# mtumalan/VisionTransformer

Measured on AMD Instinct MI355X. Metric: images/sec (512×512) ViT-B/16 seg, 1/2/4/8 MI355X + mask argmax match, higher is better.
Workload: dtype f32

## Files before the change

### visiontransformer_amd/csrc/common.hpp

```cpp
#pragma once
#include <hip/hip_runtime.h>
#include <stdint.h>

#include "../../include/vitseg.h"

namespace vitseg {

constexpr int WAVE = 64;

typedef float f32x4 __attribute__((ext_vector_type(4)));
typedef float f32x16 __attribute__((ext_vector_type(16)));
typedef short bf16x8 __attribute__((ext_vector_type(8)));
typedef short bf16x4 __attribute__((ext_vector_type(4)));

void set_error(const char* fmt, ...);
int hip_fail(hipError_t e, const char* what);

enum Opt {
    OPT_NO_F32P = 0,
    OPT_NO_P8,
    OPT_NO_H16P,
    OPT_NO_RAGGED_P8,
    OPT_NO_DROPMASK,
    OPT_DROPW_LIMIT_MB,
    OPT_UPSAMPLE_GLOBAL,
    OPT_BF16_TILES,
    OPT_F32P_NOINL,
    OPT_GN,
    OPT_NO_MASK2,
    OPT_NO_SMALL,
    OPT_SMALL_VARIANT,
    OPT_SMALL_MAX_ROWS,
    OPT_CONV_DMA,
    OPT_COUNT
};
long opt(int id);

#define VITSEG_CHECK_ARG(cond, code, ...) \
    do {                                  \
        if (!(cond)) {                    \
            ::vitseg::set_error(__VA_ARGS__); \
            return (code);                \
        }                                 \
    } while (0)

#define VITSEG_LAUNCH_CHECK(what)                               \
    do {                                                        \
        hipError_t e__ = hipGetLastError();                     \
        if (e__ != hipSuccess) return ::vitseg::hip_fail(e__, what); \
    } while (0)

inline size_t up256(size_t v) { return (v + 255) & ~(size_t)255; }

__device__ __forceinline__ int xcd_remap(int bid, int nwg) {
    const int q = nwg >> 3, r = nwg & 7, xcd = bid & 7, idx = bid >> 3;
    const int base = (xcd < r) ? xcd * (q + 1) : r * (q + 1) + (xcd - r) * q;
    return base + idx;
}

struct AttnTile {
    int rt, head, b;
};
__device__ __forceinline__ AttnTile attn_tile(int ntiles, int A) {
    const int t = xcd_remap(blockIdx.x, gridDim.x);
    const int bh = t / ntiles;
    AttnTile r;
// ... 118 lines not shown
#endif
__device__ __forceinline__ int wave_sum(int v) {
    for (int d = WAVE / 2; d > 0; d >>= 1) v += __shfl_xor(v, d);
    return v;
}

__device__ __forceinline__ float gelu_phi(float u) {
#pragma clang fp contract(off)
    const float a = fabsf(u) * 0.70710678118654752440f;
    const float c = fminf(a, 5.0f);
    float q = __uint_as_float(0xb6e5811du);
    q = fmaf(c, q, __uint_as_float(0x38d55d79u));
    q = fmaf(c, q, __uint_as_float(0xba2329bbu));
    q = fmaf(c, q, __uint_as_float(0x3ae4efa2u));
    q = fmaf(c, q, __uint_as_float(0x3a233c25u));
    q = fmaf(c, q, __uint_as_float(0xbce796e6u));
    q = fmaf(c, q, __uint_as_float(0x3e181a64u));
    q = fmaf(c, q, __uint_as_float(0x3f6b1c07u));
    q = fmaf(c, q, __uint_as_float(0x3fd05f5fu));
    const float e = __builtin_amdgcn_exp2f(-(a * q));
    return u >= 0.f ? fmaf(e, -0.5f, 1.0f) : 0.5f * e;
}
__device__ __forceinline__ float gelu_erf(float u) {
#pragma clang fp contract(off)
    return u * gelu_phi(u);
}

__device__ __forceinline__ float gelu_erf_grad(float u) {
#pragma clang fp contract(off)
    const float pdf = __builtin_amdgcn_exp2f((u * u) * -0.72134752044448170368f);
    return fmaf(u * pdf, 0.39894228040143267794f, gelu_phi(u));
}

__device__ __forceinline__ float gelu_erf_fast(float u) {
    const float x = fabsf(u) * 0.70710678118654752440f;
    float t = fmaf(x, 0.0000430638f, 0.0002765672f);
    t = fmaf(x, t, 0.0001520143f);
    t = fmaf(x, t, 0.0092705272f);
    t = fmaf(x, t, 0.0422820123f);
    t = fmaf(x, t, 0.0705230784f);
    t = fmaf(x, t, 1.0f);
    t = t * t;
    t = t * t;
    t = t * t;
    t = t * t;
    const float erf_abs = 1.0f - __builtin_amdgcn_rcpf(t);
    return 0.5f * u + 0.5f * fabsf(u) * erf_abs;
}
struct GeluPair {
    float g, d;
};
__device__ __forceinline__ GeluPair gelu_erf_pair_fast(float u) {
    const float a = fabsf(u) * 0.70710678118654752440f;
    const float c = fminf(a, 4.5f);
    float q = __uint_as_float(0xb98ef51du);
    q = fmaf(c, q, __uint_as_float(0x3b8f4085u));
    q = fmaf(c, q, __uint_as_float(0xbd04359fu));
    q = fmaf(c, q, __uint_as_float(0x3e1a8172u));
    q = fmaf(c, q, __uint_as_float(0x3f6af0d8u));
    q = fmaf(c, q, __uint_as_float(0x3fd0616eu));
    const float e = __builtin_amdgcn_exp2f(-(a * q));
    const float phi = u >= 0.f ? fmaf(e, -0.5f, 1.0f) : 0.5f * e;
    const float pdf = __builtin_amdgcn_exp2f((u * u) * -0.72134752044448170368f);
    return GeluPair{u * phi, fmaf(u * pdf, 0.39894228040143267794f, phi)};
}

__device__ __forceinline__ unsigned short f32_to_bf16(float f) {
    unsigned u = __float_as_uint(f);
    if ((u & 0x7fffffffu) > 0x7f800000u) return (unsigned short)((u >> 16) | 0x40);
    return (unsigned short)((u + 0x7fffu + ((u >> 16) & 1u)) >> 16);
}
__device__ __forceinline__ unsigned pack2_bf16(float lo, float hi) {
    typedef __bf16 bf16v2_t __attribute__((ext_vector_type(2)));
    typedef float f32v2_t __attribute__((ext_vector_type(2)));
    const f32v2_t f = {lo, hi};
    return __builtin_bit_cast(unsigned, __builtin_convertvector(f, bf16v2_t));
}
__device__ __forceinline__ float bf16_to_f32(unsigned short h) { return __uint_as_float(((unsigned)h) << 16); }

typedef unsigned short bf16_t;
// ... 31 lines not shown
```

### visiontransformer_amd/csrc/gemm_dispatch.hip

```cpp
#include "gemm_tiles.hpp"

namespace vitseg {
namespace {

int whole_split_shape(int M, int N, int K, int kstep) { return K % kstep == 0 ? whole_split(M, N, K, kstep) : 0; }

int thin_slices(int K, int kstep) {
    if (K < 256 || K % kstep != 0) return 0;
    const int sl = K / kstep / 4;
    return sl > THIN_MAX_SPLITS ? THIN_MAX_SPLITS : sl < 1 ? 1 : sl;
}

int whole_split_applies(const GemmArgs& a, int epi, int kstep) {
    const int sp = whole_split_shape(a.M, a.N, a.K, kstep);
    const bool ok = sp && a.thin_scratch && (size_t)sp * a.M * a.N <= a.thin_capacity && !a.drop.thresh &&
                    !a.aux && a.splitk <= 1 && a.ldc % 4 == 0 && (epi == EPI_BIAS || epi == EPI_GELU || epi == EPI_RESADD);
    return ok ? sp : 0;
}

int thin_split_applies(const GemmArgs& a, int epi, int kstep) {
    const bool h16 = kstep == 64;
    const int sl = thin_slices(a.K, kstep);
    const bool ok = sl && a.thin_scratch && a.thin_rows > 0 && a.thin_rows <= THIN_MAX_ROWS && a.M > a.thin_rows &&
                    (size_t)sl * a.thin_rows * a.N <= a.thin_capacity && (a.M - a.thin_rows) % BM == 0 &&
                    (h16 || (!a.drop.thresh && !a.aux)) && a.splitk <= 1 && a.ldc % 4 == 0 &&
                    (epi == EPI_BIAS || epi == EPI_GELU || epi == EPI_RESADD || (h16 && epi == EPI_DGELU));
    return ok ? sl : 0;
}

template <typename F>
int sliced(GemmArgs a, int splits, float* scratch, hipStream_t s, F launch) {
    float* out = (float*)a.C;
    if (splits > 1) {
        a.C = scratch;
        a.splitk = splits;
    }
    a.split_stride = (size_t)a.M * a.N;
    if (int rc = launch(a)) return rc;
    return splits > 1 ? launch_splitk_reduce(scratch, out, (size_t)a.M * a.N / 4, splits, s) : VITSEG_OK;
}

enum H16Kernel { HK_NONE, HK_TILE, HK_LARGE, HK_XL, HK_P8, HK_H16P };

struct H16Route {
    H16Kernel body;
    int body_rows;
    int tail_rows;
    int slices;
    int colsum_rows;
};

}

int launch_gemm_f32(const GemmArgs& a_in, int amode, int epi, hipStream_t s, int x3) {
    if (x3 != 1 && x3 != 2) x3 = 0;
    GemmArgs a = a_in;
    if (amode == A_PLAIN) {
        if (const int sp = whole_split_applies(a_in, epi, 32)) {
            a.thin_rows = a_in.M;
            return launch_thin_rows(GT_F32, x3, a, epi, sp, s);
        }
        if (const int sl = thin_split_applies(a_in, epi, 32)) {
            if (int rc = launch_thin_rows(GT_F32, x3, a_in, epi, sl, s)) return rc;
            a.M = a_in.M - a_in.thin_rows;
        }
    }
    a.thin_scratch = nullptr;
    VITSEG_CHECK_ARG(a.M > 0 && a.N > 0 && a.K > 0 && a.K % 4 == 0, VITSEG_EINVAL, "gemm_f32: bad M/N/K %d %d %d", a.M, a.N, a.K);
    VITSEG_CHECK_ARG(a.N % 4 == 0 && a.ldc % 4 == 0, VITSEG_ESHAPE, "gemm: N=%d and ldc=%d must be multiples of 4", a.N, a.ldc);
    if (amode == A_PLAIN) {
        VITSEG_CHECK_ARG(a.lda % 4 == 0, VITSEG_EINVAL, "gemm_f32: lda %% 4");
        if (!x3 && gemm_f32p_applies(a, epi)) return launch_gemm_f32p(a, epi, s);
    } else if (amode == A_PATCH && epi == EPI_POS) {
        VITSEG_CHECK_ARG(a.P % 4 == 0, VITSEG_ESHAPE, "patch size must be a multiple of 4");
    } else if (amode == A_CONV3 && epi == EPI_RELU) {
        VITSEG_CHECK_ARG(a.D % 4 == 0, VITSEG_ESHAPE, "hidden size must be a multiple of 4");
    }
    static const char* const who[3] = {"gemm_f32", "gemm_f32 (x3)", "gemm_f32 (x3, split W)"};
    return launch_gemm_tile(GT_F32, true, amode, epi, x3, a, s, who[x3]);
}

int launch_gemm_f32_bwd(const GemmArgs& a, int amode, int ta, int tb, int epi, hipStream_t s) {
    VITSEG_CHECK_ARG(a.M > 0 && a.N > 0 && a.K > 0, VITSEG_EINVAL, "gemm_bwd: bad M/N/K %d %d %d", a.M, a.N, a.K);
    VITSEG_CHECK_ARG(a.N % 4 == 0 && a.ldc % 4 == 0 && a.lda % 4 == 0 && a.ldw % 4 == 0, VITSEG_ESHAPE,
                     "gemm_bwd: leading dimensions must be multiples of 4");
    VITSEG_CHECK_ARG(ta || a.K % 4 == 0, VITSEG_ESHAPE, "gemm_bwd: K %% 4");
    VITSEG_CHECK_ARG(!ta || a.M % 4 == 0, VITSEG_ESHAPE, "gemm_bwd: M %% 4 for a T-form A");
    return launch_gemm_tile_bwd(amode, ta, tb, epi, a, s);
}

int launch_wgrad_f32(GemmArgs a, float* scratch, hipStream_t s) {
    const int splits = wgrad_splits(a.M, a.N, a.K, 32);
    VITSEG_CHECK_ARG(splits <= 1 || (a.ldc == a.N && scratch), VITSEG_EINVAL, "wgrad: split-K needs a dense output and scratch");
    return sliced(a, splits, scratch, s, [&](const GemmArgs& g) { return launch_gemm_f32_bwd(g, A_PLAIN, 1, 1, EPI_BIAS, s); });
}

static int route_h16(const GemmArgs& a_in, int amode, int epi, H16Route& r) {
    r = H16Route{HK_NONE, 0, 0, 0, 0};
    const bool want_cs = a_in.colsum_out && a_in.colsum_scratch && epi == EPI_DGELU;
    const auto persistent = [&](const GemmArgs& g) {
        r.body = gemm_h16p_applies(g, epi) ? HK_H16P : HK_P8;
        r.body_rows = g.M;
        r.colsum_rows = want_cs ? g.M : 0;
        return VITSEG_OK;
    };
    GemmArgs a = a_in;
    if (amode == A_PLAIN) {
        if (const int sp = whole_split_applies(a_in, epi, 64)) {
            r.tail_rows = a_in.M;
            r.slices = sp;
            return VITSEG_OK;
        }
        if (a_in.M % 256 != 0 && a_in.M % 256 <= 128 && gemm_p8_applies(a_in, epi) &&
            gemm_p8_rounds(a_in.M, a_in.N) == gemm_p8_rounds(a_in.M - a_in.M % 256, a_in.N) && !opt(OPT_NO_RAGGED_P8))
            return persistent(a_in);
        const int sl = (a_in.M - a_in.thin_rows) % LBM == 0 ? thin_split_applies(a_in, epi, 64) : 0;
        if (sl) {
            r.tail_rows = a_in.thin_rows;
            r.slices = sl;
            a.M = a_in.M - a_in.thin_rows;
        }
    }
    VITSEG_CHECK_ARG(a.M > 0 && a.N > 0 && a.K > 0, VITSEG_EINVAL, "gemm_bf16: bad M/N/K %d %d %d", a.M, a.N, a.K);
    VITSEG_CHECK_ARG(a.K % 64 == 0, VITSEG_ESHAPE, "gemm_bf16: K=%d must be a multiple of 64", a.K);
    VITSEG_CHECK_ARG(a.N % 4 == 0 && a.ldc % 4 == 0, VITSEG_ESHAPE, "gemm: N=%d and ldc=%d must be multiples of 4", a.N, a.ldc);
    if (amode == A_PLAIN && gemm_p8_applies(a, epi)) {
        const int tail = a.M % 256;
        if (tail != 0 && tail <= 128) {
            r.tail_rows = tail;
            a.M -= tail;
        }
        return persistent(a);
    }
    const long force = opt(OPT_BF16_TILES);
    const bool xl = force ? force == 3 : (a.M >= 8192 && a.N >= 2048);
    const bool large = force ? force == 2 : (!xl && a.M >= 4096 && a.K >= 2048);
    r.body_rows = a.M;
    if (amode == A_PLAIN) {
        VITSEG_CHECK_ARG(a.lda % 8 == 0, VITSEG_EINVAL, "gemm_bf16: lda %% 8");
        r.body = xl ? HK_XL : large ? HK_LARGE : HK_TILE;
        if (epi == EPI_BIAS || epi == EPI_GELU || epi == EPI_DGELU || epi == EPI_RESADD) return VITSEG_OK;
    } else if (amode == A_CONV3 && (epi == EPI_RELU || epi == EPI_BIAS)) {
        VITSEG_CHECK_ARG(a.D % 64 == 0 && a.zeros, VITSEG_ESHAPE, "%s must be a multiple of 64",
                         epi == EPI_RELU ? "hidden size" : "channel count");
        r.body = large ? HK_LARGE : HK_TILE;
        return VITSEG_OK;
    }
    set_error("gemm_bf16: unsupported amode/epilogue %d/%d", amode, epi);
    return VITSEG_EINVAL;
}

int launch_gemm_bf16(const GemmArgs& a_in, int amode, int epi, hipStream_t s, bool f16) {
    H16Route r;
    if (int rc = route_h16(a_in, amode, epi, r)) return rc;
    const GemmType type = f16 ? GT_F16 : GT_BF16;
    const bool out_f32 = epi == EPI_RESADD || amode == A_CONV3;
    GemmArgs a = a_in;
    if (r.slices) {
        a.thin_rows = r.tail_rows;
        if (int rc = launch_thin_rows(type, 0, a, epi, r.slices, s)) return rc;
    }
    a.M = r.body_rows;
    a.thin_scratch = nullptr;
    if (!r.colsum_rows) a.colsum_scratch = nullptr;
    int rc = VITSEG_OK;
    switch (r.body) {
        case HK_NONE: break;
        case HK_P8: rc = launch_gemm_p8(a, epi, s, f16); break;
        case HK_H16P: rc = launch_gemm_h16p(a, s, f16); break;
        case HK_XL: rc = launch_gemm_large(f16, amode, epi, 256, a, s, "gemm_bf16"); break;
        case HK_LARGE: rc = launch_gemm_large(f16, amode, epi, 128, a, s, "gemm_bf16"); break;
        case HK_TILE: rc = launch_gemm_tile(type, out_f32, amode, epi, 0, a, s, "gemm_bf16");
    }
    if (rc) return rc;
    if (r.tail_rows && !r.slices) {
        GemmArgs t = a;
        const auto row = [&](const void* p, size_t esz) { return (char*)p + (size_t)r.body_rows * a.ldc * esz; };
        t.M = r.tail_rows;
        t.row_base = a.row_base + r.body_rows;
        t.A = (const char*)a.A + (size_t)r.body_rows * a.lda * 2;
        if (a.aux) t.aux = row(a.aux, 2);
        if (a.R) t.R = (const float*)row(a.R, epi == EPI_RESADD ? 4 : 2);
        t.C = row(a.C, out_f32 ? 4 : 2);
        if ((rc = launch_gemm_tile(type, out_f32, A_PLAIN, epi, 0, t, s, "gemm_bf16"))) return rc;
    }
    if (!a_in.colsum_out) return VITSEG_OK;
    VITSEG_CHECK_ARG(a_in.colsum_scratch && !f16, VITSEG_EINVAL, "gemm: column sums need bf16 + scratch");
    if (r.colsum_rows > 0)
        return launch_colsum_finish_fused((const bf16_t*)a_in.C + (size_t)r.colsum_rows * a_in.ldc, a_in.M - r.colsum_rows,
                                          2 * ((r.colsum_rows + 255) / 256), a_in.colsum_out, a_in.colsum_scratch, a_in.N,
                                          a_in.ldc, s);
    return launch_colsum(a_in.C, 1, a_in.colsum_out, a_in.colsum_scratch, a_in.M, a_in.N, a_in.ldc, s);
}
// ... 37 lines not shown
```

### visiontransformer_amd/csrc/gemm_tile.hip

```cpp
#include "gemm_tiles.hpp"

namespace vitseg {
namespace {

template <typename T> struct Elem;
template <> struct Elem<float> { static constexpr int CE = 4, BKE = 32; };
template <> struct Elem<bf16_t> { static constexpr int CE = 8, BKE = 64; };
template <> struct Elem<f16_t> { static constexpr int CE = 8, BKE = 64; };

template <typename T>
struct ARow {
    const T* base;
    int y, x;
    bool valid;
};

template <typename T, int AMODE>
__device__ __forceinline__ ARow<T> make_arow(const GemmArgs& p, int m) {
    ARow<T> r;
    r.valid = m < p.M;
    r.y = r.x = 0;
    const T* A = (const T*)p.A;
    if (!r.valid) {
        r.base = A;
// ... 134 lines not shown
                wrow[i] = (const T*)p.W + (size_t)(wvalid[i] ? n : 0) * p.ldw;
            }
        }
        const bool ta_col_ok = m0 + tc * 4 < p.M, tb_col_ok = n0 + tc * 4 < p.N;
        f32x4 ra[4], rb[4];
        bool oka[4], okb[4];
        auto gload = [&](int kt) {
            const int k = (kt + kt0) * BKE + lc * CE;
            const int kc = min(k, p.K - CE);
#pragma unroll
            for (int i = 0; i < 4; ++i) {
                if constexpr (TA) {
                    const int kr = (kt + kt0) * BKE + tr + 8 * i;
                    oka[i] = ta_col_ok && kr < p.K;
                    ra[i] = *(const f32x4*)((const T*)p.A + (size_t)(oka[i] ? kr : 0) * p.lda +
                                            (oka[i] ? m0 + tc * 4 : 0));
                } else {
                    ra[i] = load_a<T, AMODE>(p, arow[i], k, oka[i]);
                }
                if constexpr (TB) {
                    const int kr = (kt + kt0) * BKE + tr + 8 * i;
                    okb[i] = tb_col_ok && kr < p.K;
                    rb[i] = *(const f32x4*)((const T*)p.W + (size_t)(okb[i] ? kr : 0) * p.ldw +
                                            (okb[i] ? n0 + tc * 4 : 0));
                } else {
                    rb[i] = *(const f32x4*)(wrow[i] + kc);
                    okb[i] = wvalid[i] && k < p.K;
                }
            }
        };
        const int wpos = lr * BK + ((lc ^ ((lr >> 1) & 7)) << 2);
        const int tpos = tr * BM + tc * 4;
        const int xpos = lr * 16 + ((((lc >> 1) ^ ((lr >> 1) & 3)) << 2) | ((lc & 1) << 1));
        auto split = [&](const f32x4& v, uint2& hi, uint2& lo) {
            const _Float16 h0 = (_Float16)v[0], h1 = (_Float16)v[1], h2 = (_Float16)v[2], h3 = (_Float16)v[3];
            hi.x = __builtin_bit_cast(unsigned, f16x2{h0, h1});
            hi.y = __builtin_bit_cast(unsigned, f16x2{h2, h3});
            lo.x = H16<f16_t>::pack2((v[0] - (float)h0) * 2048.f, (v[1] - (float)h1) * 2048.f);
            lo.y = H16<f16_t>::pack2((v[2] - (float)h2) * 2048.f, (v[3] - (float)h3) * 2048.f);
        };
        auto swrite = [&](int buf) {
            const f32x4 z = {0.f, 0.f, 0.f, 0.f};
#pragma unroll
            for (int i = 0; i < 4; ++i) {
                if constexpr (X3) {
                    uint2 hi, lo;
                    split(oka[i] ? ra[i] : z, hi, lo);
                    *(uint2*)&lds[buf][0][xpos + 32 * i * 16] = hi;
                    *(uint2*)&lds[buf][0][2048 + xpos + 32 * i * 16] = lo;
                    if constexpr (X3 == 2) {
                        const f32x4 w = okb[i] ? rb[i] : z;
                        hi = uint2{__float_as_uint(w[0]), __float_as_uint(w[1])};
                        lo = uint2{__float_as_uint(w[2]), __float_as_uint(w[3])};
                    } else {
                        split(okb[i] ? rb[i] : z, hi, lo);
                    }
                    *(uint2*)&lds[buf][1][xpos + 32 * i * 16] = hi;
                    *(uint2*)&lds[buf][1][2048 + xpos + 32 * i * 16] = lo;
                } else {
                    *(f32x4*)&lds[buf][0][TA ? tpos + 8 * i * BM : wpos + 32 * i * BK] = oka[i] ? ra[i] : z;
                    *(f32x4*)&lds[buf][1][TB ? tpos + 8 * i * BN : wpos + 32 * i * BK] = okb[i] ? rb[i] : z;
                }
            }
        };
        if constexpr (X3) {
            f32x4 ah[2][MI], al[2][MI], bh[2][NI], bl[2][NI];
            const int xsw = (li >> 1) & 3;
            auto lfragx = [&](int buf, int st, int slot) {
                const int ch = ((2 * st + lh) ^ xsw) << 2;
#pragma unroll
                for (int mi = 0; mi < MI; ++mi) {
                    const float* r = &lds[buf][0][(a_row0 + li + mi * 32) * 16 + ch];
                    ah[slot][mi] = *(const f32x4*)r;
                    al[slot][mi] = *(const f32x4*)(r + 2048);
                }
#pragma unroll
                for (int ni = 0; ni < NI; ++ni) {
                    const float* r = &lds[buf][1][(b_col0 + li + ni * 32) * 16 + ch];
                    bh[slot][ni] = *(const f32x4*)r;
                    bl[slot][ni] = *(const f32x4*)(r + 2048);
                }
            };
            auto mfmax = [&](int slot) {
#pragma unroll
                for (int mi = 0; mi < MI; ++mi)
#pragma unroll
                    for (int ni = 0; ni < NI; ++ni) {
                        const bf16x8 xh = __builtin_bit_cast(bf16x8, ah[slot][mi]), xl = __builtin_bit_cast(bf16x8, al[slot][mi]);
// ... 243 lines not shown
    else if (rows_valid <= 64)
        gemm_tile<T, OutT, AMODE, EPI, 2, 1, TA, TB, X3>(p, lds, m0, n0, 0, wave * 32);
    else
        gemm_tile<T, OutT, AMODE, EPI, 2, 2, TA, TB, X3>(p, lds, m0, n0, (wave >> 1) * 64, (wave & 1) * 64);
}

template <typename T, typename OutT, int AMODE, int EPI, int TA = 0, int TB = 0, int X3 = 0>
int launch_one(GemmArgs a, hipStream_t s) {
    if (a.ldw == 0) a.ldw = TB ? a.N : a.K;
    if (!a.gn) a.gn = env_gn();
    const int tiles = ((a.M + BM - 1) / BM) * ((a.N + BN - 1) / BN);
    const int splits = a.splitk > 1 ? a.splitk : 1;
    hipLaunchKernelGGL((gemm_kernel<T, OutT, AMODE, EPI, TA, TB, X3>), dim3(tiles, splits), dim3(256), 0, s, a);
    VITSEG_LAUNCH_CHECK("gemm");
    return VITSEG_OK;
}

template <int EPI, typename OutT>
__global__ __launch_bounds__(256) void thin_reduce_kernel(const float* __restrict__ partial, const float* __restrict__ bias,
                                                          const float* __restrict__ R, OutT* __restrict__ C, int rows, int N,
                                                          int ldc, int splits, OutT* __restrict__ aux, DropArgs drop,
                                                          unsigned row0) {
    const int n4 = N >> 2;
    const int i = blockIdx.x * 256 + threadIdx.x;
    if (i >= rows * n4) return;
    const int r = i / n4, c = (i - r * n4) * 4;
    const size_t slab = (size_t)rows * N;
    f32x4 acc = *(const f32x4*)(partial + (size_t)r * N + c);
    for (int sIdx = 1; sIdx < splits; ++sIdx) {
        const f32x4 v = *(const f32x4*)(partial + sIdx * slab + (size_t)r * N + c);
#pragma unroll
        for (int e = 0; e < 4; ++e) acc[e] += v[e];
    }
    f32x4 b4 = {0.f, 0.f, 0.f, 0.f};
    if (bias) b4 = *(const f32x4*)(bias + c);
    f32x4 res = {0.f, 0.f, 0.f, 0.f};
    if (EPI == EPI_RESADD) res = *(const f32x4*)(R + (size_t)r * ldc + c);
    if constexpr (EPI == EPI_DGELU) {
        const uint2 d = *(const uint2*)((const OutT*)R + (size_t)r * ldc + c);
        res[0] = H16<OutT>::lo(d.x);
        res[1] = H16<OutT>::hi(d.x);
        res[2] = H16<OutT>::lo(d.y);
        res[3] = H16<OutT>::hi(d.y);
    }
    f32x4 der = {0.f, 0.f, 0.f, 0.f};
    const unsigned key = drop.thresh ? drop_key(drop.seed, drop.stream, row0 + (unsigned)r) : 0u;
#pragma unroll
    for (int e = 0; e < 4; ++e) {
        float x = acc[e] + b4[e];
        if (EPI == EPI_GELU) {
            if (sizeof(OutT) == 4) x = gelu_erf(x);
            else if (aux) { const GeluPair gp = gelu_erf_pair_fast(x); x = gp.g; der[e] = gp.d; }
            else x = gelu_erf_fast(x);
        }
        if (EPI == EPI_RESADD) {
            if (drop.thresh) x = drop_keep(key, (unsigned)(c + e), drop.thresh) ? x * drop.scale : 0.f;
            x = res[e] + x;
        }
        if (EPI == EPI_DGELU) x *= res[e];
        acc[e] = x;
    }
    if constexpr (sizeof(OutT) == 4) {
        *(f32x4*)(C + (size_t)r * ldc + c) = acc;
    } else {
        uint2 h;
        h.x = H16<OutT>::pack2(acc[0], acc[1]);
        h.y = H16<OutT>::pack2(acc[2], acc[3]);
        *(uint2*)(C + (size_t)r * ldc + c) = h;
        if (EPI == EPI_GELU && aux) {
            h.x = H16<OutT>::pack2(der[0], der[1]);
            h.y = H16<OutT>::pack2(der[2], der[3]);
            *(uint2*)(aux + (size_t)r * ldc + c) = h;
        }
    }
}

template <typename OutT>
int launch_thin_reduce(const GemmArgs& a, int epi, int splits, hipStream_t s) {
    const int rows = a.thin_rows, body = a.M - rows;
    const int blocks = (rows * (a.N / 4) + 255) / 256;
    const float* R = nullptr;
    if (a.R) R = epi == EPI_DGELU ? (const float*)((const OutT*)a.R + (size_t)body * a.ldc) : a.R + (size_t)body * a.ldc;
    OutT* C = (OutT*)a.C + (size_t)body * a.ldc;
    OutT* aux = a.aux ? (OutT*)a.aux + (size_t)body * a.ldc : nullptr;
    const unsigned row0 = (unsigned)(a.row_base + body);
#define VITSEG_THIN(E)                                                                                                 \
    hipLaunchKernelGGL((thin_reduce_kernel<E, OutT>), dim3(blocks), dim3(256), 0, s, a.thin_scratch, a.bias, R, C, rows, \
                       a.N, a.ldc, splits, aux, a.drop, row0)
    switch (epi) {
        case EPI_BIAS: VITSEG_THIN(EPI_BIAS); break;
        case EPI_GELU: VITSEG_THIN(EPI_GELU); break;
        case EPI_DGELU:
            if constexpr (sizeof(OutT) == 4) {
                set_error("thin_reduce: dGELU epilogue is 16-bit only");
                return VITSEG_EINVAL;
            } else {
                VITSEG_THIN(EPI_DGELU);
            }
            break;
        default: VITSEG_THIN(EPI_RESADD);
    }
#undef VITSEG_THIN
    VITSEG_LAUNCH_CHECK("thin_reduce");
    return VITSEG_OK;
}

}

int launch_gemm_tile(GemmType type, bool out_f32, int amode, int epi, int x3, const GemmArgs& a, hipStream_t s, const char* who) {
#define ROW(ID, T, OutT, AMODE, EPI, X3) \
    if (type == ID && out_f32 == (sizeof(OutT) == 4) && amode == AMODE && epi == EPI && x3 == X3) return launch_one<T, OutT, AMODE, EPI, 0, 0, X3>(a, s);
#define ROW_X3(AMODE, EPI) ROW(GT_F32, float, float, AMODE, EPI, 0) ROW(GT_F32, float, float, AMODE, EPI, 1) ROW(GT_F32, float, float, AMODE, EPI, 2)
#define ROW_H16(AMODE, EPI) ROW(GT_BF16, bf16_t, bf16_t, AMODE, EPI, 0) ROW(GT_F16, f16_t, f16_t, AMODE, EPI, 0)
#define ROW_H16_F32(AMODE, EPI) ROW(GT_BF16, bf16_t, float, AMODE, EPI, 0) ROW(GT_F16, f16_t, float, AMODE, EPI, 0)
    ROW_X3(A_PLAIN, EPI_BIAS) ROW_X3(A_PLAIN, EPI_GELU) ROW_X3(A_PLAIN, EPI_RESADD) ROW(GT_F32, float, float, A_PLAIN, EPI_RELU, 0)
    ROW_X3(A_PATCH, EPI_POS) ROW_X3(A_CONV3, EPI_RELU)
    ROW_H16(A_PLAIN, EPI_BIAS) ROW_H16(A_PLAIN, EPI_GELU) ROW_H16(A_PLAIN, EPI_DGELU)
    ROW_H16_F32(A_PLAIN, EPI_RESADD) ROW_H16_F32(A_PLAIN, EPI_BIAS) ROW_H16_F32(A_CONV3, EPI_RELU) ROW_H16_F32(A_CONV3, EPI_BIAS)
#undef ROW_H16_F32
#undef ROW_H16
#undef ROW_X3
#undef ROW
    set_error("%s: unsupported amode/epilogue %d/%d", who, amode, epi);
    return VITSEG_EINVAL;
}

int launch_gemm_tile_bwd(int amode, int ta, int tb, int epi, const GemmArgs& a, hipStream_t s) {
    if (amode == A_PLAIN && !ta && tb && epi == EPI_BIAS) return launch_one<float, float, A_PLAIN, EPI_BIAS, 0, 1>(a, s);
    if (amode == A_PLAIN && !ta && tb && epi == EPI_DGELU) return launch_one<float, float, A_PLAIN, EPI_DGELU, 0, 1>(a, s);
    if (amode == A_PLAIN && ta && tb && epi == EPI_BIAS) return launch_one<float, float, A_PLAIN, EPI_BIAS, 1, 1>(a, s);
    if (amode == A_CONV3 && !ta && !tb && epi == EPI_BIAS) return launch_one<float, float, A_CONV3, EPI_BIAS, 0, 0>(a, s);
    set_error("gemm_bwd: unsupported combination amode %d ta %d tb %d epi %d", amode, ta, tb, epi);
    return VITSEG_EINVAL;
}

int launch_thin_rows(GemmType type, int x3, const GemmArgs& a, int epi, int slices, hipStream_t s) {
    const int rows = a.thin_rows, body = a.M - rows;
    GemmArgs t = a;
    t.A = (const char*)a.A + (size_t)body * a.lda * (type == GT_F32 ? 4 : 2);
    t.M = rows;
    t.bias = nullptr;
    t.R = nullptr;
    t.C = a.thin_scratch;
    t.ldc = a.N;
    t.splitk = slices;
    t.split_stride = (size_t)rows * a.N;
    t.thin_scratch = nullptr;
    if (type != GT_F32) {
        t.aux = nullptr;
        t.drop = DropArgs{};
    }
    if (int rc = launch_gemm_tile(type, true, A_PLAIN, EPI_BIAS, x3, t, s, "gemm (K slices)")) return rc;
    if (type == GT_F32 || epi == EPI_RESADD) return launch_thin_reduce<float>(a, epi, slices, s);
    return type == GT_F16 ? launch_thin_reduce<f16_t>(a, epi, slices, s) : launch_thin_reduce<bf16_t>(a, epi, slices, s);
}

}
```

### visiontransformer_amd/csrc/gemm_tiles.hpp

```cpp
#pragma once
#include "kernels.hpp"

namespace vitseg {

constexpr int BM = 128, BN = 128;
constexpr int BKF = 32;
constexpr int LBM = 256;
inline int env_gn() { return (int)opt(OPT_GN); }

enum GemmType { GT_F32 = 0, GT_BF16 = 1, GT_F16 = 2 };
int launch_gemm_tile(GemmType type, bool out_f32, int amode, int epi, int x3, const GemmArgs& a, hipStream_t s, const char* who);
int launch_gemm_tile_bwd(int amode, int ta, int tb, int epi, const GemmArgs& a, hipStream_t s);
int launch_thin_rows(GemmType type, int x3, const GemmArgs& a, int epi, int slices, hipStream_t s);
int launch_gemm_large(bool f16, int amode, int epi, int lbn, const GemmArgs& a, hipStream_t s, const char* who);
int launch_gemm_tt(const GemmArgs& a, hipStream_t s);
int wgrad_splits(int M, int N, int K, int kstep);

}
```

### visiontransformer_amd/csrc/vitseg_api.hip

```cpp
#include <ctype.h>
#include <stdarg.h>
#include <stdio.h>
#include <stdlib.h>
#include <strings.h>

#include <atomic>

#include <vector>

#include "kernels.hpp"
#include "profile.hpp"
#include "forward.hpp"

namespace vitseg {

static thread_local char g_err[512] = "";

void set_error(const char* fmt, ...) {
    va_list ap;
    va_start(ap, fmt);
    vsnprintf(g_err, sizeof(g_err), fmt, ap);
    va_end(ap);
}

int hip_fail(hipError_t e, const char* what) {
    set_error("%s: %s", what, hipGetErrorString(e));
    return VITSEG_EHIP;
}

static const char* const g_opt_names[OPT_COUNT] = {"no_f32p", "no_p8", "no_h16p", "no_ragged_p8", "no_dropmask",
                                                   "dropw_limit_mb", "upsample_global", "bf16_tiles", "f32p_noinl", "gn", "no_mask2", "no_small",
                                                   "small_variant", "small_max_rows", "conv_dma"};
static std::atomic<long> g_opts[OPT_COUNT];
static int opt_index(const char* name) {
    if (!name) return -1;
    for (int i = 0; i < OPT_COUNT; ++i)
        if (!strcasecmp(name, g_opt_names[i])) return i;
    return -1;
}
static long opt_parse(int id, const char* text) {
    if (id == OPT_BF16_TILES && (text[0] == 's' || text[0] == 'l' || text[0] == 'x')) return text[0] == 's' ? 1 : text[0] == 'l' ? 2 : 3;
    char* end = nullptr;
    const long v = strtol(text, &end, 10);
    if (end != text) return v;
    return (id == OPT_DROPW_LIMIT_MB || id == OPT_GN || id == OPT_SMALL_VARIANT || id == OPT_SMALL_MAX_ROWS || id == OPT_BF16_TILES) ? 0 : 1;
}
static const bool g_opts_loaded = [] {
    for (int i = 0; i < OPT_COUNT; ++i) {
        char env[64] = "VITSEG_";
        for (size_t k = 0; g_opt_names[i][k] && k + 8 < sizeof(env); ++k) {
            env[7 + k] = (char)toupper((unsigned char)g_opt_names[i][k]);
            env[8 + k] = 0;
        }
        const char* e = getenv(env);
        g_opts[i].store(e ? opt_parse(i, e) : (i == OPT_DROPW_LIMIT_MB ? -1 : 0), std::memory_order_relaxed);
    }
    return true;
}();
long opt(int id) { return g_opts[id].load(std::memory_order_relaxed); }

namespace {

using namespace plan;

struct Plan {
// ... 632 lines not shown
```

Measured before the change: 615.5.

## Fuse thin-row split-K GEMM and its reduce into one ticketed launch

Adds a fused thin-rows kernel. Each block computes one K slice of a 64-column tile with per-wave MFMA and writes the partial sum to scratch. The last-arriving block, found through an atomic ticket counter, then reduces all slices and applies the bias/GELU/residual epilogue. This replaces the separate slice GEMM launch and reduce launch for the tail rows, cutting launch overhead and a kernel boundary. The cost is a per-device ticket buffer, agent-scope fences and a serialized final reduction in one block per tile. The epilogue is factored into a shared helper, and GELU in the thin path uses an explicit fma.

```diff
diff --git a/visiontransformer_amd/csrc/common.hpp b/visiontransformer_amd/csrc/common.hpp
--- a/visiontransformer_amd/csrc/common.hpp
+++ b/visiontransformer_amd/csrc/common.hpp
@@ -32,6 +32,7 @@
     OPT_SMALL_VARIANT,
     OPT_SMALL_MAX_ROWS,
     OPT_CONV_DMA,
+    OPT_NO_THIN_FUSED,
     OPT_COUNT
 };
 long opt(int id);
@@ -216,7 +217,7 @@
     return fmaf(u * pdf, 0.39894228040143267794f, gelu_phi(u));
 }
 
-__device__ __forceinline__ float gelu_erf_fast(float u) {
+__device__ __forceinline__ float gelu_erf_fast_abs(float u) {
     const float x = fabsf(u) * 0.70710678118654752440f;
     float t = fmaf(x, 0.0000430638f, 0.0002765672f);
     t = fmaf(x, t, 0.0001520143f);
@@ -228,8 +229,16 @@
     t = t * t;
     t = t * t;
     t = t * t;
-    const float erf_abs = 1.0f - __builtin_amdgcn_rcpf(t);
+    return 1.0f - __builtin_amdgcn_rcpf(t);
+}
+__device__ __forceinline__ float gelu_erf_fast(float u) {
+    const float erf_abs = gelu_erf_fast_abs(u);
     return 0.5f * u + 0.5f * fabsf(u) * erf_abs;
+}
+__device__ __forceinline__ float gelu_erf_fast_thin(float u) {
+#pragma clang fp contract(off)
+    const float erf_abs = gelu_erf_fast_abs(u);
+    return fmaf(0.5f * fabsf(u), erf_abs, 0.5f * u);
 }
 struct GeluPair {
     float g, d;
diff --git a/visiontransformer_amd/csrc/gemm_dispatch.hip b/visiontransformer_amd/csrc/gemm_dispatch.hip
--- a/visiontransformer_amd/csrc/gemm_dispatch.hip
+++ b/visiontransformer_amd/csrc/gemm_dispatch.hip
@@ -28,6 +28,13 @@
     return ok ? sl : 0;
 }
 
+bool thin_fused_applies(const GemmArgs& a, int epi, int esz) {
+    const int ldw = a.ldw ? a.ldw : a.K;
+    return !opt(OPT_NO_THIN_FUSED) && !a.aux && !a.drop.thresh && a.N % 4 == 0 && a.N <= THIN_FUSED_MAX_N &&
+           (size_t)a.lda * esz % 16 == 0 && (size_t)ldw * esz % 16 == 0 &&
+           (epi == EPI_BIAS || epi == EPI_GELU || epi == EPI_RESADD);
+}
+
 template <typename F>
 int sliced(GemmArgs a, int splits, float* scratch, hipStream_t s, F launch) {
     float* out = (float*)a.C;
@@ -47,6 +54,7 @@
     int body_rows;
     int tail_rows;
     int slices;
+    bool fused;
     int colsum_rows;
 };
 
@@ -58,10 +66,10 @@
     if (amode == A_PLAIN) {
         if (const int sp = whole_split_applies(a_in, epi, 32)) {
             a.thin_rows = a_in.M;
-            return launch_thin_rows(GT_F32, x3, a, epi, sp, s);
+            return launch_thin_rows(GT_F32, x3, a, epi, sp, false, s);
         }
         if (const int sl = thin_split_applies(a_in, epi, 32)) {
-            if (int rc = launch_thin_rows(GT_F32, x3, a_in, epi, sl, s)) return rc;
+            if (int rc = launch_thin_rows(GT_F32, x3, a_in, epi, sl, thin_fused_applies(a_in, epi, 4), s)) return rc;
             a.M = a_in.M - a_in.thin_rows;
         }
     }
@@ -96,7 +104,7 @@
 }
 
 static int route_h16(const GemmArgs& a_in, int amode, int epi, H16Route& r) {
-    r = H16Route{HK_NONE, 0, 0, 0, 0};
+    r = H16Route{HK_NONE, 0, 0, 0, false, 0};
     const bool want_cs = a_in.colsum_out && a_in.colsum_scratch && epi == EPI_DGELU;
     const auto persistent = [&](const GemmArgs& g) {
         r.body = gemm_h16p_applies(g, epi) ? HK_H16P : HK_P8;
@@ -118,6 +126,7 @@
         if (sl) {
             r.tail_rows = a_in.thin_rows;
             r.slices = sl;
+            r.fused = thin_fused_applies(a_in, epi, 2);
             a.M = a_in.M - a_in.thin_rows;
         }
     }
@@ -158,7 +167,7 @@
     GemmArgs a = a_in;
     if (r.slices) {
         a.thin_rows = r.tail_rows;
-        if (int rc = launch_thin_rows(type, 0, a, epi, r.slices, s)) return rc;
+        if (int rc = launch_thin_rows(type, 0, a, epi, r.slices, r.fused, s)) return rc;
     }
     a.M = r.body_rows;
     a.thin_scratch = nullptr;
diff --git a/visiontransformer_amd/csrc/gemm_thin.hip b/visiontransformer_amd/csrc/gemm_thin.hip
--- /dev/null
+++ b/visiontransformer_amd/csrc/gemm_thin.hip
@@ -0,0 +1,257 @@
+#include <atomic>
+#include <mutex>
+
+#include "gemm_tiles.hpp"
+
+namespace vitseg {
+namespace {
+
+constexpr int THIN_TICKET_SETS = 32;
+
+struct ThinArgs {
+    const void* A;
+    const void* W;
+    float* scratch;
+    const float* bias;
+    const float* R;
+    void* C;
+    unsigned* tickets;
+    int rows, N, K, lda, ldw, ldc, epi;
+};
+
+template <typename T, int X3>
+__global__ __launch_bounds__(256) void thin_fused_kernel(const ThinArgs p) {
+    constexpr int BKE = sizeof(T) == 4 ? 32 : 64;
+    const int tid = threadIdx.x, lane = tid & 63, wave = tid >> 6;
+    const int li = lane & 31, lh = lane >> 5;
+    const int n0 = blockIdx.x * THIN_BN;
+    const int S = gridDim.y, slice = blockIdx.y;
+    const int KT_all = p.K / BKE;
+    const int kt0 = (int)((long long)KT_all * slice / S);
+    const int KT = (int)((long long)KT_all * (slice + 1) / S) - kt0;
+    const int row0 = (wave >> 1) * 32, col0 = n0 + (wave & 1) * 32;
+    __shared__ __attribute__((aligned(16))) float xpose[4][2][32 * 32];
+
+    if (row0 < p.rows && col0 < p.N) {
+        f32x16 acc, acc1;
+#pragma unroll
+        for (int r = 0; r < 16; ++r) acc[r] = acc1[r] = 0.f;
+        const int lr = lane >> 3, lc = lane & 7;
+        const char *ap[4], *wp[4];
+#pragma unroll
+        for (int i = 0; i < 4; ++i) {
+            const int r = lr + 8 * i;
+            ap[i] = (const char*)p.A + ((size_t)min(row0 + r, p.rows - 1) * p.lda + (size_t)kt0 * BKE) * sizeof(T) + lc * 16;
+            wp[i] = (const char*)p.W + ((size_t)min(col0 + r, p.N - 1) * p.ldw + (size_t)kt0 * BKE) * sizeof(T) + lc * 16;
+        }
+        float* const la = &xpose[wave][0][0];
+        float* const lw = &xpose[wave][1][0];
+        const auto fchunk = [&](int i) { return X3 ? 4 * (i >> 1) + 2 * lh + (i & 1) : 2 * i + lh; };
+        struct Stage {
+            f32x4 a[2][4], b[2][4];
+        };
+        const auto load = [&](Stage& st, int kt) {
+#pragma unroll
+            for (int u = 0; u < 2; ++u) {
+                const size_t off = (size_t)min(kt + u, KT - 1) * 128;
+#pragma unroll
+                for (int i = 0; i < 4; ++i) {
+                    st.b[u][i] = *(const f32x4*)(wp[i] + off);
+                    st.a[u][i] = *(const f32x4*)(ap[i] + off);
+                }
+            }
+        };
+        const auto step = [&](const Stage& st, int u) {
+            f32x4 fa[4], fb[4];
+#pragma unroll
+            for (int i = 0; i < 4; ++i) {
+                const int r = lr + 8 * i, pos = r * 32 + ((lc ^ ((r >> 1) & 7)) << 2);
+                *(f32x4*)&la[pos] = st.a[u][i];
+                *(f32x4*)&lw[pos] = st.b[u][i];
+            }
+            __builtin_amdgcn_fence(__ATOMIC_ACQ_REL, "wavefront");
+            __builtin_amdgcn_wave_barrier();
+#pragma unroll
+            for (int i = 0; i < 4; ++i) {
+                const int pos = li * 32 + ((fchunk(i) ^ ((li >> 1) & 7)) << 2);
+                fa[i] = *(const f32x4*)&la[pos];
+                fb[i] = *(const f32x4*)&lw[pos];
+            }
+            __builtin_amdgcn_fence(__ATOMIC_ACQ_REL, "wavefront");
+            __builtin_amdgcn_wave_barrier();
+            if constexpr (X3) {
+#pragma unroll
+                for (int h = 0; h < 2; ++h) {
+                    uint2 h0, l0, h1, l1;
+                    x3_split(fa[2 * h], h0, l0);
+                    x3_split(fa[2 * h + 1], h1, l1);
+                    const bf16x8 xh = __builtin_bit_cast(bf16x8, uint4{h0.x, h0.y, h1.x, h1.y});
+                    const bf16x8 xl = __builtin_bit_cast(bf16x8, uint4{l0.x, l0.y, l1.x, l1.y});
+                    const f32x4 w0 = fb[2 * h], w1 = fb[2 * h + 1];
+                    if constexpr (X3 == 2) {
+                        h0 = uint2{__float_as_uint(w0[0]), __float_as_uint(w0[1])};
+                        l0 = uint2{__float_as_uint(w0[2]), __float_as_uint(w0[3])};
+                        h1 = uint2{__float_as_uint(w1[0]), __float_as_uint(w1[1])};
+                        l1 = uint2{__float_as_uint(w1[2]), __float_as_uint(w1[3])};
+                    } else {
+                        x3_split(w0, h0, l0);
+                        x3_split(w1, h1, l1);
+                    }
+                    const bf16x8 yh = __builtin_bit_cast(bf16x8, uint4{h0.x, h0.y, h1.x, h1.y});
+                    const bf16x8 yl = __builtin_bit_cast(bf16x8, uint4{l0.x, l0.y, l1.x, l1.y});
+                    acc = H16<f16_t>::mfma(xh, yh, acc);
+                    acc1 = H16<f16_t>::mfma(xl, yh, acc1);
+                    acc1 = H16<f16_t>::mfma(xh, yl, acc1);
+                }
+            } else if constexpr (sizeof(T) == 4) {
+#pragma unroll
+                for (int j = 0; j < 4; ++j)
+#pragma unroll
+                    for (int e = 0; e < 4; ++e)
+                        acc = __builtin_amdgcn_mfma_f32_32x32x2f32(fa[j][e], fb[j][e], acc, 0, 0, 0);
+            } else {
+#pragma unroll
+                for (int j = 0; j < 4; ++j)
+                    acc = H16<T>::mfma(__builtin_bit_cast(bf16x8, fa[j]), __builtin_bit_cast(bf16x8, fb[j]), acc);
+            }
+        };
+        Stage s0, s1;
+        load(s0, 0);
+        for (int kt = 0; kt < KT; kt += 4) {
+            const bool more = kt + 2 < KT;
+            if (more) load(s1, kt + 2);
+            step(s0, 0);
+            if (kt + 1 < KT) step(s0, 1);
+            if (kt + 4 < KT) load(s0, kt + 4);
+            if (more) {
+                step(s1, 0);
+                if (kt + 3 < KT) step(s1, 1);
+            }
+        }
+        if constexpr (X3) {
+#pragma unroll
+            for (int r = 0; r < 16; ++r) acc[r] = fmaf(acc1[r], 1.0f / 2048.0f, acc[r]);
+        }
+        float* out = p.scratch + (size_t)slice * p.rows * p.N;
+        const int col = col0 + li;
+#pragma unroll
+        for (int r = 0; r < 16; ++r) {
+            const int row = row0 + (r & 3) + 8 * (r >> 2) + 4 * lh;
+            if (row < p.rows && col < p.N) out[(size_t)row * p.N + col] = acc[r] + 0.f;
+        }
+    }
+
+    __shared__ unsigned s_ticket;
+    __builtin_amdgcn_s_waitcnt(0x0F70);
+    __syncthreads();
+    if (tid == 0) {
+        __builtin_amdgcn_fence(__ATOMIC_RELEASE, "agent");
+        const unsigned t = __hip_atomic_fetch_add(p.tickets + blockIdx.x, 1u, __ATOMIC_RELAXED, __HIP_MEMORY_SCOPE_AGENT);
+        if (t == (unsigned)(S - 1)) __builtin_amdgcn_fence(__ATOMIC_ACQUIRE, "agent");
+        s_ticket = t;
+    }
+    __syncthreads();
+    if (s_ticket != (unsigned)(S - 1)) return;
+
+    const size_t slab = (size_t)p.rows * p.N;
+    const int items = p.rows * (THIN_BN / 4);
+    for (int i0 = tid; i0 < items; i0 += 512) {
+        f32x4 v[2][THIN_MAX_SPLITS];
+        int r[2], c[2];
+        bool ok[2];
+#pragma unroll
+        for (int q = 0; q < 2; ++q) {
+            const int i = i0 + 256 * q;
+            r[q] = i / (THIN_BN / 4);
+            c[q] = n0 + (i % (THIN_BN / 4)) * 4;
+            ok[q] = i < items && c[q] < p.N;
+            const float* src = p.scratch + (ok[q] ? (size_t)r[q] * p.N + c[q] : 0);
+#pragma unroll
+            for (int sl = 0; sl < THIN_MAX_SPLITS; ++sl)
+                v[q][sl] = *(const f32x4*)(src + min(sl, S - 1) * slab);
+        }
+#pragma unroll
+        for (int q = 0; q < 2; ++q) {
+            if (!ok[q]) continue;
+            f32x4 acc = v[q][0];
+#pragma unroll
+            for (int sl = 1; sl < THIN_MAX_SPLITS; ++sl)
+                if (sl < S) {
+#pragma unroll
+                    for (int e = 0; e < 4; ++e) acc[e] += v[q][sl][e];
+                }
+            const DropArgs nodrop{};
+            using OutT = T;
+            if (p.epi == EPI_RESADD) thin_epilogue<EPI_RESADD, float>(acc, p.bias, p.R, (float*)p.C, nullptr, p.ldc, r[q], c[q], nodrop, 0u);
+            else if (p.epi == EPI_GELU) thin_epilogue<EPI_GELU, OutT>(acc, p.bias, p.R, (OutT*)p.C, nullptr, p.ldc, r[q], c[q], nodrop, 0u);
+            else thin_epilogue<EPI_BIAS, OutT>(acc, p.bias, p.R, (OutT*)p.C, nullptr, p.ldc, r[q], c[q], nodrop, 0u);
+        }
+    }
+    if (tid == 0) __hip_atomic_store(p.tickets + blockIdx.x, 0u, __ATOMIC_RELAXED, __HIP_MEMORY_SCOPE_AGENT);
+}
+
+unsigned* ticket_set() {
+    static std::mutex mu;
+    static unsigned* base[64] = {};
+    static std::atomic<unsigned> next{0};
+    int dev = 0;
+    if (hipGetDevice(&dev) != hipSuccess || dev < 0 || dev >= 64) return nullptr;
+    {
+        std::lock_guard<std::mutex> lock(mu);
+        if (!base[dev]) {
+            unsigned* b = nullptr;
+            const size_t bytes = (size_t)THIN_TICKET_SETS * THIN_TICKETS * sizeof(unsigned);
+            if (hipMalloc((void**)&b, bytes) != hipSuccess) return nullptr;
+            if (hipMemset(b, 0, bytes) != hipSuccess || hipDeviceSynchronize() != hipSuccess) {
+                (void)hipFree(b);
+                return nullptr;
+            }
+            base[dev] = b;
+        }
+    }
+    return base[dev] + (size_t)(next.fetch_add(1u, std::memory_order_relaxed) % THIN_TICKET_SETS) * THIN_TICKETS;
+}
+
+}
+
+int launch_thin_fused(GemmType type, int x3, const GemmArgs& a, int epi, int slices, hipStream_t s) {
+    const int rows = a.thin_rows, body = a.M - rows;
+    const int tiles = (a.N + THIN_BN - 1) / THIN_BN;
+    const size_t esz = type == GT_F32 ? 4 : 2;
+    const int kstep = 128 / (int)esz;
+    VITSEG_CHECK_ARG(rows > 0 && rows <= THIN_MAX_ROWS && body >= 0 && slices >= 1 && slices <= THIN_MAX_SPLITS &&
+                         a.K % kstep == 0 && a.K / kstep >= slices && tiles <= THIN_TICKETS && a.N % 4 == 0 && a.thin_scratch &&
+                         !a.aux && !a.drop.thresh && (epi == EPI_BIAS || epi == EPI_GELU || epi == EPI_RESADD),
+                     VITSEG_EINVAL, "gemm (thin rows, one launch): rows %d slices %d N %d K %d epilogue %d", rows, slices, a.N,
+                     a.K, epi);
+    const bool out_f32 = type == GT_F32 || epi == EPI_RESADD;
+    ThinArgs t;
+    t.A = (const char*)a.A + (size_t)body * a.lda * esz;
+    t.W = a.W;
+    t.scratch = a.thin_scratch;
+    t.bias = a.bias;
+    t.R = a.R ? a.R + (size_t)body * a.ldc : nullptr;
+    t.C = (char*)a.C + (size_t)body * a.ldc * (out_f32 ? 4 : 2);
+    t.rows = rows;
+    t.N = a.N;
+    t.K = a.K;
+    t.lda = a.lda;
+    t.ldw = a.ldw ? a.ldw : a.K;
+    t.ldc = a.ldc;
+    t.epi = epi;
+    t.tickets = ticket_set();
+    if (!t.tickets) {
+        set_error("gemm (thin rows, one launch): no device memory for the tickets");
+        return VITSEG_EHIP;
+    }
+    const dim3 grid(tiles, slices), block(256);
+    if (type == GT_BF16) hipLaunchKernelGGL((thin_fused_kernel<bf16_t, 0>), grid, block, 0, s, t);
+    else if (type == GT_F16) hipLaunchKernelGGL((thin_fused_kernel<f16_t, 0>), grid, block, 0, s, t);
+    else if (x3 == 1) hipLaunchKernelGGL((thin_fused_kernel<float, 1>), grid, block, 0, s, t);
+    else if (x3 == 2) hipLaunchKernelGGL((thin_fused_kernel<float, 2>), grid, block, 0, s, t);
+    else hipLaunchKernelGGL((thin_fused_kernel<float, 0>), grid, block, 0, s, t);
+    VITSEG_LAUNCH_CHECK("gemm (thin rows, one launch)");
+    return VITSEG_OK;
+}
+
+}
diff --git a/visiontransformer_amd/csrc/gemm_tile.hip b/visiontransformer_amd/csrc/gemm_tile.hip
--- a/visiontransformer_amd/csrc/gemm_tile.hip
+++ b/visiontransformer_amd/csrc/gemm_tile.hip
@@ -190,20 +190,13 @@
         const int wpos = lr * BK + ((lc ^ ((lr >> 1) & 7)) << 2);
         const int tpos = tr * BM + tc * 4;
         const int xpos = lr * 16 + ((((lc >> 1) ^ ((lr >> 1) & 3)) << 2) | ((lc & 1) << 1));
-        auto split = [&](const f32x4& v, uint2& hi, uint2& lo) {
-            const _Float16 h0 = (_Float16)v[0], h1 = (_Float16)v[1], h2 = (_Float16)v[2], h3 = (_Float16)v[3];
-            hi.x = __builtin_bit_cast(unsigned, f16x2{h0, h1});
-            hi.y = __builtin_bit_cast(unsigned, f16x2{h2, h3});
-            lo.x = H16<f16_t>::pack2((v[0] - (float)h0) * 2048.f, (v[1] - (float)h1) * 2048.f);
-            lo.y = H16<f16_t>::pack2((v[2] - (float)h2) * 2048.f, (v[3] - (float)h3) * 2048.f);
-        };
         auto swrite = [&](int buf) {
             const f32x4 z = {0.f, 0.f, 0.f, 0.f};
 #pragma unroll
             for (int i = 0; i < 4; ++i) {
                 if constexpr (X3) {
                     uint2 hi, lo;
-                    split(oka[i] ? ra[i] : z, hi, lo);
+                    x3_split(oka[i] ? ra[i] : z, hi, lo);
                     *(uint2*)&lds[buf][0][xpos + 32 * i * 16] = hi;
                     *(uint2*)&lds[buf][0][2048 + xpos + 32 * i * 16] = lo;
                     if constexpr (X3 == 2) {
@@ -211,7 +204,7 @@
                         hi = uint2{__float_as_uint(w[0]), __float_as_uint(w[1])};
                         lo = uint2{__float_as_uint(w[2]), __float_as_uint(w[3])};
                     } else {
-                        split(okb[i] ? rb[i] : z, hi, lo);
+                        x3_split(okb[i] ? rb[i] : z, hi, lo);
                     }
                     *(uint2*)&lds[buf][1][xpos + 32 * i * 16] = hi;
                     *(uint2*)&lds[buf][1][2048 + xpos + 32 * i * 16] = lo;
@@ -521,47 +514,7 @@
 #pragma unroll
         for (int e = 0; e < 4; ++e) acc[e] += v[e];
     }
-    f32x4 b4 = {0.f, 0.f, 0.f, 0.f};
-    if (bias) b4 = *(const f32x4*)(bias + c);
-    f32x4 res = {0.f, 0.f, 0.f, 0.f};
-    if (EPI == EPI_RESADD) res = *(const f32x4*)(R + (size_t)r * ldc + c);
-    if constexpr (EPI == EPI_DGELU) {
-        const uint2 d = *(const uint2*)((const OutT*)R + (size_t)r * ldc + c);
-        res[0] = H16<OutT>::lo(d.x);
-        res[1] = H16<OutT>::hi(d.x);
-        res[2] = H16<OutT>::lo(d.y);
-        res[3] = H16<OutT>::hi(d.y);
-    }
-    f32x4 der = {0.f, 0.f, 0.f, 0.f};
-    const unsigned key = drop.thresh ? drop_key(drop.seed, drop.stream, row0 + (unsigned)r) : 0u;
-#pragma unroll
-    for (int e = 0; e < 4; ++e) {
-        float x = acc[e] + b4[e];
-        if (EPI == EPI_GELU) {
-            if (sizeof(OutT) == 4) x = gelu_erf(x);
-            else if (aux) { const GeluPair gp = gelu_erf_pair_fast(x); x = gp.g; der[e] = gp.d; }
-            else x = gelu_erf_fast(x);
-        }
-        if (EPI == EPI_RESADD) {
-            if (drop.thresh) x = drop_keep(key, (unsigned)(c + e), drop.thresh) ? x * drop.scale : 0.f;
-            x = res[e] + x;
-        }
-        if (EPI == EPI_DGELU) x *= res[e];
-        acc[e] = x;
-    }
-    if constexpr (sizeof(OutT) == 4) {
-        *(f32x4*)(C + (size_t)r * ldc + c) = acc;
-    } else {
-        uint2 h;
-        h.x = H16<OutT>::pack2(acc[0], acc[1]);
-        h.y = H16<OutT>::pack2(acc[2], acc[3]);
-        *(uint2*)(C + (size_t)r * ldc + c) = h;
-        if (EPI == EPI_GELU && aux) {
-            h.x = H16<OutT>::pack2(der[0], der[1]);
-            h.y = H16<OutT>::pack2(der[2], der[3]);
-            *(uint2*)(aux + (size_t)r * ldc + c) = h;
-        }
-    }
+    thin_epilogue<EPI, OutT>(acc, bias, R, C, aux, ldc, r, c, drop, row0);
 }
 
 template <typename OutT>
@@ -623,7 +576,8 @@
     return VITSEG_EINVAL;
 }
 
-int launch_thin_rows(GemmType type, int x3, const GemmArgs& a, int epi, int slices, hipStream_t s) {
+int launch_thin_rows(GemmType type, int x3, const GemmArgs& a, int epi, int slices, bool fused, hipStream_t s) {
+    if (fused) return launch_thin_fused(type, x3, a, epi, slices, s);
     const int rows = a.thin_rows, body = a.M - rows;
     GemmArgs t = a;
     t.A = (const char*)a.A + (size_t)body * a.lda * (type == GT_F32 ? 4 : 2);
diff --git a/visiontransformer_amd/csrc/gemm_tiles.hpp b/visiontransformer_amd/csrc/gemm_tiles.hpp
--- a/visiontransformer_amd/csrc/gemm_tiles.hpp
+++ b/visiontransformer_amd/csrc/gemm_tiles.hpp
@@ -11,9 +11,65 @@
 enum GemmType { GT_F32 = 0, GT_BF16 = 1, GT_F16 = 2 };
 int launch_gemm_tile(GemmType type, bool out_f32, int amode, int epi, int x3, const GemmArgs& a, hipStream_t s, const char* who);
 int launch_gemm_tile_bwd(int amode, int ta, int tb, int epi, const GemmArgs& a, hipStream_t s);
-int launch_thin_rows(GemmType type, int x3, const GemmArgs& a, int epi, int slices, hipStream_t s);
+int launch_thin_rows(GemmType type, int x3, const GemmArgs& a, int epi, int slices, bool fused, hipStream_t s);
+constexpr int THIN_BN = 64, THIN_TICKETS = 256, THIN_FUSED_MAX_N = THIN_BN * THIN_TICKETS;
+int launch_thin_fused(GemmType type, int x3, const GemmArgs& a, int epi, int slices, hipStream_t s);
 int launch_gemm_large(bool f16, int amode, int epi, int lbn, const GemmArgs& a, hipStream_t s, const char* who);
 int launch_gemm_tt(const GemmArgs& a, hipStream_t s);
 int wgrad_splits(int M, int N, int K, int kstep);
 
+__device__ __forceinline__ void x3_split(const f32x4& v, uint2& hi, uint2& lo) {
+    const _Float16 h0 = (_Float16)v[0], h1 = (_Float16)v[1], h2 = (_Float16)v[2], h3 = (_Float16)v[3];
+    hi.x = __builtin_bit_cast(unsigned, f16x2{h0, h1});
+    hi.y = __builtin_bit_cast(unsigned, f16x2{h2, h3});
+    lo.x = H16<f16_t>::pack2((v[0] - (float)h0) * 2048.f, (v[1] - (float)h1) * 2048.f);
+    lo.y = H16<f16_t>::pack2((v[2] - (float)h2) * 2048.f, (v[3] - (float)h3) * 2048.f);
 }
+
+template <int EPI, typename OutT>
+__device__ __forceinline__ void thin_epilogue(f32x4 acc, const float* __restrict__ bias, const float* R, OutT* C, OutT* aux,
+                                              int ldc, int r, int c, const DropArgs& drop, unsigned row0) {
+    f32x4 b4 = {0.f, 0.f, 0.f, 0.f};
+    if (bias) b4 = *(const f32x4*)(bias + c);
+    f32x4 res = {0.f, 0.f, 0.f, 0.f};
+    if (EPI == EPI_RESADD) res = *(const f32x4*)(R + (size_t)r * ldc + c);
+    if constexpr (EPI == EPI_DGELU) {
+        const uint2 d = *(const uint2*)((const OutT*)R + (size_t)r * ldc + c);
+        res[0] = H16<OutT>::lo(d.x);
+        res[1] = H16<OutT>::hi(d.x);
+        res[2] = H16<OutT>::lo(d.y);
+        res[3] = H16<OutT>::hi(d.y);
+    }
+    f32x4 der = {0.f, 0.f, 0.f, 0.f};
+    const unsigned key = drop.thresh ? drop_key(drop.seed, drop.stream, row0 + (unsigned)r) : 0u;
+#pragma unroll
+    for (int e = 0; e < 4; ++e) {
+        float x = acc[e] + b4[e];
+        if (EPI == EPI_GELU) {
+            if (sizeof(OutT) == 4) x = gelu_erf(x);
+            else if (aux) { const GeluPair gp = gelu_erf_pair_fast(x); x = gp.g; der[e] = gp.d; }
+            else x = gelu_erf_fast_thin(x);
+        }
+        if (EPI == EPI_RESADD) {
+            if (drop.thresh) x = drop_keep(key, (unsigned)(c + e), drop.thresh) ? x * drop.scale : 0.f;
+            x = res[e] + x;
+        }
+        if (EPI == EPI_DGELU) x *= res[e];
+        acc[e] = x;
+    }
+    if constexpr (sizeof(OutT) == 4) {
+        *(f32x4*)(C + (size_t)r * ldc + c) = acc;
+    } else {
+        uint2 h;
+        h.x = H16<OutT>::pack2(acc[0], acc[1]);
+        h.y = H16<OutT>::pack2(acc[2], acc[3]);
+        *(uint2*)(C + (size_t)r * ldc + c) = h;
+        if (EPI == EPI_GELU && aux) {
+            h.x = H16<OutT>::pack2(der[0], der[1]);
+            h.y = H16<OutT>::pack2(der[2], der[3]);
+            *(uint2*)(aux + (size_t)r * ldc + c) = h;
+        }
+    }
+}
+
+}
diff --git a/visiontransformer_amd/csrc/vitseg_api.hip b/visiontransformer_amd/csrc/vitseg_api.hip
--- a/visiontransformer_amd/csrc/vitseg_api.hip
+++ b/visiontransformer_amd/csrc/vitseg_api.hip
@@ -30,7 +30,7 @@
 
 static const char* const g_opt_names[OPT_COUNT] = {"no_f32p", "no_p8", "no_h16p", "no_ragged_p8", "no_dropmask",
                                                    "dropw_limit_mb", "upsample_global", "bf16_tiles", "f32p_noinl", "gn", "no_mask2", "no_small",
-                                                   "small_variant", "small_max_rows", "conv_dma"};
+                                                   "small_variant", "small_max_rows", "conv_dma", "no_thin_fused"};
 static std::atomic<long> g_opts[OPT_COUNT];
 static int opt_index(const char* name) {
     if (!name) return -1;
```

Result: no change. 615.1 (-0.1%).
